# tyb311/TCCT

Measured on AMD Instinct MI355X. Metric: OCT B-scans/sec fwd+bwd(+clip+AdamW), stc_tt bs=8 1x800x1100, higher is better.
Workload: dtype bf16; 1 GPU; stc_tt --los=di bs=8/GPU 1x800x1100 (net tensors 3x800x1104); global_batch=8, parallelism=dp1, ranks=1, grad_allreduce=none, slowest_step=88

## Files before the change

include/tcct_hip.h:

```cpp
#ifndef TCCT_HIP_H
#define TCCT_HIP_H
#include <stdint.h>
#ifdef __cplusplus
extern "C" {
#endif

typedef void* tcct_stream_t;

enum { TCCT_F32 = 0, TCCT_BF16 = 1 };
enum { TCCT_ACT_NONE = 0, TCCT_ACT_LRELU = 1, TCCT_ACT_HSWISH = 2, TCCT_ACT_GELU = 3, TCCT_ACT_SIGMOID = 4,
       TCCT_ACT_ABS = 5 };
enum { TCCT_CRIT_DICE = 0, TCCT_CRIT_DICE2 = 1, TCCT_CRIT_IOU = 2, TCCT_CRIT_MSE = 3 };
enum { TCCT_MCRIT_DICE = 0, TCCT_MCRIT_DICE2 = 1, TCCT_MCRIT_IOU = 2, TCCT_MCRIT_CE = 3 };

int tcct_version(void);
const char* tcct_last_error(void);
int tcct_set_outputs_prezeroed(int on);

int tcct_image_to_nhwc4(const float* img, void* out, int N, int Csrc, int H, int Wsrc, int Wdst, int dtype,
                        tcct_stream_t stream);
int tcct_u8_gather2d(const uint8_t* src, uint8_t* dst, int N, int SH, int SW, int C, int sy0, int sx0, int sh, int sw, int DH, int DW,
                     int dy0, int dx0, int dh, int dw, int flipy, int flipx, int mul, int div, int fill, tcct_stream_t stream);
int tcct_onehot_to_index(const int64_t* onehot, uint8_t* lab, int N, int C, int64_t HW, tcct_stream_t stream);
int tcct_labels_to_u8(const int64_t* lab, uint8_t* out, int N, int H, int Wsrc, int Wdst, tcct_stream_t stream);
// ... 129 lines not shown
                              int PW, int xs, int xo, int ds, int dof, int cin_total, int o_off, int i_off, tcct_stream_t stream);
int tcct_conv32x64_fwd33(const void* x, const void* wp, int wps, const float* bias, void* y, int N, int H, int W, double* stats, int pre_act, int force,
                         tcct_stream_t stream);
int tcct_conv32x64_wgrad33(const void* x, const void* dy, float* dw, float* dbias, int N, int H, int W, int force, tcct_stream_t stream);
int tcct_conv64x32_dgrad33(const void* dy, const void* wp_t, int wps, void* dx, int N, int H, int W, int force, tcct_stream_t stream);
int tcct_conv32_wgrad(const void* x, const void* dy, float* dw, float* dbias, int N, int H, int W, int KH, int KW, int PH,
                      int PW, tcct_stream_t stream);
int tcct_conv32_bwd3x3(const void* x, const void* dy, const void* wp_t, const void* dskip, void* dx, float* dw, float* dbias, int N, int H,
                       int W, tcct_stream_t stream);

int tcct_pw_fwd(const void* x, const float* w, const float* bias, void* y, int64_t M, int K, int N, int transposed,
                int out_dtype, tcct_stream_t stream);
int tcct_pw_wgrad(const void* x, const void* dy, float* dw, float* dbias, int64_t M, int K, int N, tcct_stream_t stream);
int tcct_pw_bwd(const void* x, const void* dy, const float* w, const void* res, void* dx, float* dw, float* dbias, int64_t M, int K, int N,
                tcct_stream_t stream);
int tcct_pw_bwd_cat2(const void* x1, const void* x2, const void* dy, const float* w, void* dx1, void* dx2, float* dw, int64_t M, int K, int N,
                     tcct_stream_t stream);
int tcct_pw_bwd_residual2(const void* x, const void* dy, const float* w, const void* res, void* dx_sum, void* dx_plain, float* dw, float* dbias,
                          int64_t M, int K, int N, tcct_stream_t stream);
int64_t tcct_pw_bwd_bn_supported(int K, int N, int post, int red_post, int split);
int tcct_pw_bwd_bn(const void* x, const void* x2, const void* dz, const void* y, const float* coef, int post, const float* w, const void* res,
                   void* dx, void* dx2, float* dw, float* dbias, int64_t M, int K, int N, const void* y_prev, const float* ab_prev,
                   int red_post, double* sums_prev, tcct_stream_t stream);
int tcct_pw_bwd_bn_sums(const void* x, const void* x2, const void* dz, const void* y, const double* sums, int raw, const float* mean_rstd,
                        const float* ab, float* dgamma, float* dbeta, int post, const float* w, const void* res, void* dx, void* dx2, float* dw,
                        float* dbias, int64_t M, int K, int N, const void* y_prev, const float* ab_prev, int red_post, double* sums_prev,
                        tcct_stream_t stream);
int tcct_pw_wgrad_strided(const void* x, const void* dy, int64_t ldy, float* dw, float* dbias, int64_t M, int K, int N,
                          tcct_stream_t stream);
int tcct_pw_fwd_residual(const void* x, const float* w, const float* bias, const void* res, const float* scale, int64_t per_sample,
                         void* y, void* y_plain, int64_t M, int K, int N, tcct_stream_t stream);
int tcct_pw_fwd_bnstats_xaff(const void* y_prev, const float* ab_prev, const float* w, const float* bias, void* y, int64_t M, int K, int N, double* stats,
                             tcct_stream_t stream);
int tcct_pw_bwd_bn_sums_xaff(const void* y_prev, const float* ab_prev, const void* dz, const void* y, const double* sums, int raw, const float* mean_rstd,
                             const float* ab, float* dgamma, float* dbeta, const float* w, const void* res, void* dx, float* dw, float* dbias, int64_t M,
                             int K, int N, int red_post, double* sums_prev, tcct_stream_t stream);
int tcct_pw_fwd_gelu_residual(const void* x1, const float* w, const float* bias, const void* res, const float* scale, int64_t per_sample, void* y,
                              int64_t M, int K, int N, tcct_stream_t stream);
int tcct_pw_bwd_residual2_sum(const void* x, const void* dy_a, const void* dy_b, const float* w, const void* res, void* dx_sum, void* dx_plain, float* dw,
                              float* dbias, int64_t M, int K, int N, tcct_stream_t stream);
int tcct_pw_bwd_lnb(const void* x, const void* dy, const float* w, const void* t, const float* mean_rstd, const float* gamma, const void* res, void* dt,
                    float* dw, float* dbias, float* dgamma, float* dbeta, int64_t M, int K, int N, tcct_stream_t stream);
int tcct_pw_bwd_gelu(const void* x1, const void* dy, const float* w, void* dx1, float* dw, float* dbias, int64_t M, int K, int N, tcct_stream_t stream);
int tcct_pw_dgrad_residual(const void* dy, const float* w, const void* res, void* dx_sum, void* dx_plain, int64_t M, int Nout, int K,
                           tcct_stream_t stream);
int tcct_pw_fwd_cat2(const void* x1, const void* x2, int K1, const float* w, const float* bias, void* y, int64_t M, int K, int N,
                     double* stats, int pre_act, tcct_stream_t stream);
int tcct_pw_fwd_f32_upadd(const void* x, const float* w, const float* bias, float* y, int B, int uH, int uW, int K, int N, const float* up, tcct_stream_t stream);
int tcct_pw_dgrad_split2(const void* dy, const float* w, void* dx1, void* dx2, int K1, int64_t M, int Nout, int K, tcct_stream_t stream);
int tcct_pw_bwd_cat2_bias(const void* x1, const void* x2, const void* dy, const float* w, void* dx1, void* dx2, float* dw, float* dbias, int64_t M,
                          int K, int N, tcct_stream_t stream);
int tcct_tail_compose(const float* w1, const float* b1, const float* w2, const float* b2, float* wc, float* c, tcct_stream_t stream);
int tcct_tail_compose_bwd(const float* w1, const float* b1, const float* w2, const float* dwc, const float* dc, float* dw1, float* db1, float* dw2,
                          float* db2, tcct_stream_t stream);
int tcct_tail_compose3(const float* w1, const float* b1, const float* w2, const float* b2, const float* w3, const float* b3, int C, float* wcc, float* wa,
                       float* wb, float* ccc, tcct_stream_t stream);
int tcct_tail_compose3_bwd(const float* w1, const float* b1, const float* w2, const float* b2, const float* w3, int C, const float* dwa, const float* dwb,
                           const float* dccc, float* dw1, float* db1, float* dw2, float* db2, float* dw3, float* db3, tcct_stream_t stream);
int tcct_pw_fwd_cat2_f32(const void* x1, const void* x2, int K1, const float* w, const float* bias, float* y, int64_t M, int K, int N, tcct_stream_t stream);
int tcct_head_compose(const float* wt, const float* bt, const float* wa, const float* ba, int C, float* wh, float* ch, tcct_stream_t stream);
int tcct_head_compose_bwd(const float* wt, const float* bt, const float* wa, int C, const float* dwh, const float* dch, float* dwt, float* dbt,
                          float* dwa, float* dba, tcct_stream_t stream);
int tcct_pw_wgrad_cat2(const void* x1, const void* x2, int K1, const void* dy, float* dw, float* dbias, int64_t M, int K, int N,
                       tcct_stream_t stream);
int tcct_pw_fwd_bnstats(const void* x, const float* w, const float* bias, void* y, int64_t M, int K, int N, double* stats, int pre_act,
                        tcct_stream_t stream);

int tcct_im2col3x3_c3(const void* x4, void* out, int N, int H, int W, int stride, int dtype, tcct_stream_t stream);
int tcct_c3_fwd(const void* x4, const float* w, const float* bias, void* y, int B, int H, int W, int stride, double* stats, int stat_pre,
                const float* ab, int pre_act, int post_act, tcct_stream_t stream);
int tcct_c3_wgrad(const void* x4, const void* dy, float* dw, float* dbias, int B, int H, int W, int stride, tcct_stream_t stream);
int tcct_c3_bn_fwd_train(const void* x4, const float* w, const float* bias, void* z, int B, int H, int W, int stride, double* sums,
                         const float* gamma, const float* beta, float eps, float momentum, float* running_mean, float* running_var,
                         int64_t* num_batches_tracked, float* mean_rstd, float* ab, int post_act, tcct_stream_t stream);
int tcct_c3_bn_fwd_eval(const void* x4, const float* w, const float* bias, void* z, int B, int H, int W, int stride, const float* ab, int post_act,
                        tcct_stream_t stream);
int tcct_c3_bn_bwd_reduce(const void* x4, const float* w, const float* bias, const void* dz, int B, int H, int W, int stride, const float* ab,
                          double* raw, int post_act, tcct_stream_t stream);
int tcct_c3_bn_bwd_wgrad(const void* x4, const float* w, const float* bias, const void* dz, int B, int H, int W, int stride, const float* coef,
                         float* dw, float* dbias, int post_act, tcct_stream_t stream);
int64_t tcct_c3_bn_bwd_prefetch(int tiles_ahead);
int tcct_c3_bn_bwd_onepass(const void* x4, const float* w, const float* bias, const void* dz, int B, int H, int W, int stride, const float* mean_rstd,
                           const float* ab, float* work, double* sums, float* dw, float* dbias, float* dgamma, float* dbeta, int post_act, tcct_stream_t stream);
int tcct_pw_wgrad_smalln(const void* x, const void* dy, float* dw, float* dbias, int64_t M, int K, int N, int x_dtype,
                         int dy_dtype, tcct_stream_t stream);

int tcct_stream_copy(const void* src, void* dst, int64_t nbytes, tcct_stream_t stream);

int64_t tcct_kernel_census(int which, int reset);
int tcct_marker(int id, tcct_stream_t stream);

int tcct_dwconv3x3_fwd(const void* x, const float* w, const float* bias, void* y, int N, int H, int W, int C,
                       int stride, int add_input, int dtype, tcct_stream_t stream);
int tcct_dwconv3x3_fwd_bnstats(const void* x, const float* w, const float* bias, void* y, int N, int H, int W, int C, int stride,
                               int add_input, double* stats, int dtype, tcct_stream_t stream);
int tcct_dwconv3x3_dgrad(const void* dy, const float* w, void* dx, int N, int H, int W, int C, int stride,
                         int add_input, int dtype, tcct_stream_t stream);
int tcct_dwconv3x3_dgrad_add(const void* dy, const float* w, const void* res, void* dx, int N, int H, int W, int C, int stride,
                             int add_input, int dtype, tcct_stream_t stream);
int tcct_dwconv3x3_wgrad(const void* x, const void* dy, float* dw, float* dbias, int N, int H, int W, int C,
                         int stride, int dtype, tcct_stream_t stream);
int tcct_dwconv3x3_fwd_xaff(const void* x, const float* xab, const float* w, const float* bias, void* y, int N, int H, int W, int C, int stride,
                            double* stats, int dtype, tcct_stream_t stream);
int tcct_dwconv3x3_wgrad_xaff(const void* x, const float* xab, const void* dy, float* dw, float* dbias, int N, int H, int W, int C, int stride, int dtype,
                              tcct_stream_t stream);
int tcct_dwconv3x3_dgrad_bnred(const void* dy, const float* w, const void* y_prev, const float* ab_prev, void* dx, double* raw, int N, int H, int W, int C,
                               int dtype, tcct_stream_t stream);

int tcct_metapool_fwd(const void* x, void* y, int B, int64_t N, int C, int dtype, tcct_stream_t stream);
int tcct_metapool_bwd(const void* dy, void* dx, int B, int64_t N, int C, int dtype, tcct_stream_t stream);
int tcct_metapool_residual_fwd(const void* x, const void* res, const float* scale, void* y, int B, int64_t N, int C, int dtype,
                               tcct_stream_t stream);
int tcct_metapool_scaled_bwd(const void* dy, const float* scale, void* dx, int B, int64_t N, int C, int dtype, tcct_stream_t stream);
int tcct_ln_metapool_residual_fwd(const void* t, void* y, int B, int64_t N, int C, const float* gamma, const float* beta, float eps, const float* scale,
                                  int dtype, tcct_stream_t stream);
int tcct_ln_metapool_residual_ln_fwd(const void* t, void* y, void* y2, int B, int64_t N, int C, const float* gamma, const float* beta, float eps,
                                     const float* scale, const float* gamma2, const float* beta2, float eps2, float* mean_rstd2, int dtype, tcct_stream_t stream);
int tcct_ln_metapool_residual_bwd(const void* t, const void* dy, void* dt, int B, int64_t N, int C, const float* gamma, float eps, const float* scale,
                                  float* dgamma, float* dbeta, int dtype, tcct_stream_t stream);
int tcct_maxpool2_fwd(const void* x, void* y, int N, int H, int W, int C, int dtype, tcct_stream_t stream);
int tcct_maxpool2_bwd(const void* x, const void* dy, void* dx, int N, int H, int W, int C, int dtype, tcct_stream_t stream);
int tcct_maxpool2_bwd_add(const void* x, const void* dy, const void* res, void* dx, int N, int H, int W, int C, int dtype,
                          tcct_stream_t stream);
int tcct_bilinear_fwd(const void* x, void* y, int N, int H, int W, int C, int Ho, int Wo, int align_corners, int dtype,
                      tcct_stream_t stream);
int tcct_bilinear_bwd_separable(const float* dy, float* dx, float* workspace, int N, int H, int W, int C, int Ho, int Wo,
                                int align_corners, tcct_stream_t stream);
int tcct_bilinear_add_fwd(const void* x, const void* res, void* y, int N, int H, int W, int C, int Ho, int Wo, int align_corners,
                          int dtype, tcct_stream_t stream);
int64_t tcct_bilinear_bwd_x2(int on);
int tcct_bilinear_bwd(const void* dy, void* dx, int N, int H, int W, int C, int Ho, int Wo, int align_corners, int dtype,
                      tcct_stream_t stream);
int tcct_l2norm_fwd(const void* x, void* y, int64_t M, int C, float eps, int dtype, tcct_stream_t stream);
int tcct_l2norm_bwd(const void* x, const void* dy, void* dx, int64_t M, int C, float eps, int dtype, tcct_stream_t stream);
int tcct_l2norm_bwd_scaled(const void* x, const void* dy, void* dx, int64_t M, int C, float eps, float scale, int dtype,
                           tcct_stream_t stream);
int tcct_l2norm_bwd_scaled_add(const void* x, const void* dy, const void* res, void* dx, int64_t M, int C, float eps, float scale, int dtype,
                               tcct_stream_t stream);
int tcct_normadd_fwd(const void* g0, const void* g1, const void* g2, float* inv1, float* inv2, void* out, int N, int H, int W, int C,
                     int h1, int w1, int h2, int w2, float eps, int dtype, tcct_stream_t stream);
int tcct_normadd6_fwd(const void* a0, const void* b0, const void* a1, const void* b1, const void* a2, const void* b2, float* inv1, float* inv2,
                      void* out, int N, int H, int W, int C, int h1, int w1, int h2, int w2, float eps, int dtype, tcct_stream_t stream);
int tcct_l2norm_bwd2_scaled(const void* xa, const void* xb, const void* dn, const void* res_a, const void* res_b, void* da, void* db,
                            int64_t M, int C, float eps, float scale, int dtype, tcct_stream_t stream);

int tcct_softmax_dice_fwd(const void* logits, const uint8_t* labels, int64_t M, int C, double* sums, float* loss,
                          int dtype, tcct_stream_t stream);
int tcct_softmax_dice_bwd(const void* logits, const uint8_t* labels, int64_t M, int C, const double* sums,
                          const float* grad_out, float grad_scale, void* dlogits, int dtype, tcct_stream_t stream);
int tcct_updice_fwd(const float* low, const uint8_t* labels, int B, int h, int w, int H, int W, int C, double* sums, float* loss,
                    tcct_stream_t stream);
int tcct_updice_bwd(const float* low, const uint8_t* labels, int B, int h, int w, int H, int W, int C, const double* sums,
                    const float* grad_out, float grad_scale, float* ws, float* dlow, tcct_stream_t stream);
int tcct_dice_ds_fwd(const void* logits, int dtype, const uint8_t* labels, int B, int H, int W, int C, const float* low1, int h1, int w1, const float* low2,
                     int h2, int w2, const float* low3, int h3, int w3, float coff, double* sums, float* loss, tcct_stream_t stream);
int tcct_softmax_crit_fwd(const void* logits, const uint8_t* labels, int64_t M, int C, int kind, const float* class_w, double* sums, float* loss, int dtype,
                          tcct_stream_t stream);
int tcct_softmax_crit_bwd(const void* logits, const uint8_t* labels, int64_t M, int C, int kind, const float* class_w, const double* sums, const float* grad_out,
                          float grad_scale, void* dlogits, int dtype, tcct_stream_t stream);
int tcct_upcrit_fwd(const float* low, const uint8_t* labels, int B, int h, int w, int H, int W, int C, int kind, const float* class_w, double* sums, float* loss,
                    tcct_stream_t stream);
int tcct_upcrit_bwd(const float* low, const uint8_t* labels, int B, int h, int w, int H, int W, int C, int kind, const float* class_w, const double* sums,
                    const float* grad_out, float grad_scale, float* ws, float* dlow, tcct_stream_t stream);
int tcct_crit_ds_fwd(const void* logits, int dtype, const uint8_t* labels, int B, int H, int W, int C, const float* low1, int h1, int w1, const float* low2, int h2, int w2,
                     const float* low3, int h3, int w3, float coff, int kind, const float* class_w, double* sums, float* loss, tcct_stream_t stream);
int tcct_softmax_mcrit_fwd(const void* logits, const uint8_t* labels, int B, int64_t HW, int C, int kind, const float* class_w, double* sums, float* loss, int dtype,
                           tcct_stream_t stream);
int tcct_softmax_mcrit_bwd(const void* logits, const uint8_t* labels, int B, int64_t HW, int C, int kind, const float* class_w, const double* sums, const float* grad_out,
                           float grad_scale, void* dlogits, int dtype, tcct_stream_t stream);
int tcct_upmcrit_fwd(const float* low, const uint8_t* labels, int B, int h, int w, int H, int W, int C, int kind, const float* class_w, double* sums, float* loss,
                     tcct_stream_t stream);
int tcct_upmcrit_bwd(const float* low, const uint8_t* labels, int B, int h, int w, int H, int W, int C, int kind, const float* class_w, const double* sums,
                     const float* grad_out, float grad_scale, float* ws, float* dlow, tcct_stream_t stream);
int tcct_mcrit_ds_fwd(const void* logits, int dtype, const uint8_t* labels, int B, int H, int W, int C, const float* low1, int h1, int w1, const float* low2, int h2, int w2,
                      const float* low3, int h3, int w3, float coff, int kind, const float* class_w, double* sums, float* loss, tcct_stream_t stream);
int tcct_softmax_pick(const void* logits, const uint8_t* labels, int64_t M, int C, float* prob_lab, uint8_t* argmax,
                      int dtype, tcct_stream_t stream);
int tcct_confusion_counts(const uint8_t* pred, const uint8_t* labels, int N, int64_t HW, int C, float* out,
                          tcct_stream_t stream);

int tcct_gate_fusion_fwd(const void* x1, const void* x2, const float* field, void* y, int N, int H, int W, int C, int hs, int ws,
                         int dtype, tcct_stream_t stream);
int tcct_gate_fusion_bwd(const void* dy, const float* field, void* dx1, void* dx2, int N, int H, int W, int C, int hs, int ws,
                         int dtype, tcct_stream_t stream);

int tcct_mask_boundaries(const uint8_t* mask, int32_t* out, int N, int H, int W, int C, tcct_stream_t stream);

int tcct_eval_counts(const void* pred, int pred_kind, const uint8_t* labels, int B, int H, int W, int C, int h_valid, int w_valid, int32_t* counts, int32_t* bnd_pred,
                     int32_t* bnd_lab, uint8_t* argmax, tcct_stream_t stream);
int tcct_eval_scores(const int32_t* counts, const int32_t* bnd_pred, const int32_t* bnd_lab, int B, int C, int W, int h_valid, int w_valid, double* table,
                     tcct_stream_t stream);
int tcct_ordered_decode(const void* logits, int kind, int B, int H, int W, int C, int h_valid, int w_valid, void* take_ws, uint8_t* mask, int32_t* bnd,
                        int32_t* changed, int32_t* best, tcct_stream_t stream);
int64_t tcct_layout_decode_ws_bytes(int B, int H, int W, int S, int n_free);
int tcct_layout_decode(const void* pred, int kind, int B, int H, int W, int C, const int* layers, int S, int free_mask, int h_valid, int w_valid, void* ws,
                       uint8_t* mask, int32_t* bnd, int32_t* changed, int32_t* best, uint8_t* state, tcct_stream_t stream);
int tcct_eval_layout_scores(const int32_t* counts, const int32_t* bnd_pred, const int32_t* bnd_lab, int B, int C, int S, int W, int h_valid, int w_valid,
                            double* table, tcct_stream_t stream);
int64_t tcct_layout_marginals_ws_bytes(int B, int H, int W, int S, int n_free);
int tcct_layout_marginals(const void* logits, int kind, int B, int H, int W, int C, const int* layers, int S, int free_mask, int h_valid, int w_valid, float tau,
                          void* ws, float* surf, float* var, float* logz, float* post, tcct_stream_t stream);
int tcct_eval_soft_scores(const float* surf, const float* var, const int32_t* bnd_lab, int B, int S, int W, int h_valid, int w_valid, double* table,
                          tcct_stream_t stream);
int64_t tcct_layout_nll_ws_bytes(int B, int H, int W, int S, int n_free);
int tcct_layout_nll_fwd(const void* logits, int kind, const uint8_t* t, const int32_t* bnd_lab, int B, int H, int W, int C, const int* layers, int S, int free_mask,
                        int h_valid, int w_valid, float tau, void* ws, float* nll, tcct_stream_t stream);
int tcct_layout_nll_bwd(const void* logits, int kind, const uint8_t* t, const int32_t* bnd_lab, int B, int H, int W, int C, const int* layers, int S, int free_mask,
                        int h_valid, int w_valid, float tau, const void* ws, const float* gscale, void* grad, tcct_stream_t stream);
int tcct_layout_nll_reduce(const float* nll, const int32_t* bnd_lab, int B, int S, int W, int h_valid, int w_valid, float* out, tcct_stream_t stream);

int tcct_slice_channels_fwd(const void* x, float* y, int64_t M, int C, int start, int n, int dtype, tcct_stream_t stream);
int tcct_slice_channels_bwd(const float* dy, void* dx, int64_t M, int C, int start, int n, int dtype, tcct_stream_t stream);
int tcct_label_planes(const uint8_t* labels, float* onehot, float* edge, int N, int H, int W, int start, int n,
                      tcct_stream_t stream);
int tcct_gumbel_colsoftmax_fwd(const float* x, const float* eps, float* out, float* stats, int N, int H, int W, int CH,
                               tcct_stream_t stream);
int tcct_gumbel_colsoftmax_bwd(const float* x, const float* eps, const float* stats, const float* dout, float* dx, int N,
                               int H, int W, int CH, tcct_stream_t stream);
int tcct_colsoftmax_fwd(const float* x, float* y, int N, int H, int W, tcct_stream_t stream);
int tcct_colsoftmax_bwd(const float* y, const float* dy, float* dx, int N, int H, int W, tcct_stream_t stream);
int tcct_colwsum_fwd(const float* x, const float* wts, float* out, int N, int H, int W, tcct_stream_t stream);
int tcct_colwsum_bwd(const float* dout, const float* wts, float* dx, int N, int H, int W, tcct_stream_t stream);
int tcct_mse_fwd(const float* a, const float* b, int64_t n, double* acc, float* out, tcct_stream_t stream);
int tcct_mse_bwd(const float* a, const float* b, int64_t n, const float* grad_out, float grad_scale, float* da, float* db,
                 tcct_stream_t stream);

int64_t tcct_fpl_select_workspace_bytes();
int tcct_fpl_select(const void* feat, const uint8_t* labels, const float* prob, int64_t M, int C, void* workspace, uint32_t* counts,
                    uint8_t* binmap, float* pro_sum, int dtype, tcct_stream_t stream);
int tcct_fpl_loss(const float* pro_sum, const uint32_t* counts, const float* buf_grad, int C, float* pro, float* loss, float* dpro_over_n,
                  tcct_stream_t stream);
int tcct_fpl_backward(const uint8_t* labels, const uint8_t* binmap, const float* dpro_over_n, const float* grad_out,
                      float grad_scale, int64_t M, void* dfeat, int dtype, tcct_stream_t stream);
int tcct_l2norm_bwd_fplgrad(const void* x, const uint8_t* labels, const uint8_t* binmap, const float* dpro_over_n, const float* grad_out,
                            float grad_scale, int ncls, const void* res, void* dx, int64_t M, float eps, float scale, int dtype, tcct_stream_t stream);
int tcct_bilinear_bwd_fplgrad(const uint8_t* labels, const uint8_t* binmap, const float* dpro_over_n, const float* grad_out, float grad_scale, int ncls,
                              void* dx, int N, int H, int W, int Ho, int Wo, int align_corners, int dtype, tcct_stream_t stream);
int tcct_l2norm_bwd2_fplgrad(const void* xa, const void* xb, const uint8_t* labels, const uint8_t* binmap, const float* dpro_over_n,
                             const float* grad_out, float grad_scale, int ncls, const void* res_a, const void* res_b, void* da, void* db,
                             int64_t M, float eps, float scale, int dtype, tcct_stream_t stream);

int64_t tcct_fatt_kstats_workspace_bytes(int B, int64_t N, int C);
int tcct_fatt_kstats(const void* qkv, void* workspace, float* stats, int B, int64_t N, int C, int heads, int dtype, tcct_stream_t stream);
int tcct_fatt_ktv(const void* qkv, const float* stats, float* M, int B, int64_t N, int C, int heads, int dtype, tcct_stream_t stream);
int tcct_fatt_dktv(const void* qkv, const void* dout, float* dM, float scale, int B, int64_t N, int C, int heads, int dtype,
                   tcct_stream_t stream);
int tcct_fatt_apply_fwd(const void* qkv, const float* M, const void* cv, void* out, float scale, int B, int64_t N, int C, int heads,
                        int dtype, tcct_stream_t stream);
int tcct_fatt_apply_bwd(const void* qkv, const float* stats, const float* M, const float* dM, const void* cv, const void* dout,
                        void* dqkv, void* dcv, float scale, int B, int64_t N, int C, int heads, int dtype, tcct_stream_t stream);
int tcct_dwk_strided_fwd(const void* x, int64_t ldx, const float* w, const float* bias, void* y, int64_t ldy, int B, int H, int W, int Cg,
                         int K, int flip, int accumulate, int dtype, tcct_stream_t stream);
int tcct_dwk_strided_wgrad(const void* x, int64_t ldx, const void* dy, int64_t ldy, float* dw, float* dbias, int B, int H, int W, int Cg,
                           int K, int dtype, tcct_stream_t stream);

int64_t tcct_hydra_kv_workspace_bytes(int B, int64_t N, int C);
int tcct_hydra_kv(const void* qkv, void* workspace, float* kv, int B, int64_t N, int C, int heads, int dtype, tcct_stream_t stream);
int tcct_hydra_dkv(const void* qkv, const void* dmix, void* workspace, float* dkv, float scale, int B, int64_t N, int C, int heads, int dtype,
                   tcct_stream_t stream);
int tcct_hydra_apply_fwd(const void* qkv, const float* kv, const void* cv, void* mix, float scale, int B, int64_t N, int C, int heads,
                         int dtype, tcct_stream_t stream);
int tcct_hydra_apply_bwd(const void* qkv, const float* kv, const float* dkv, const void* cv, const void* dmix, void* dqkv, void* dcv,
                         float scale, int B, int64_t N, int C, int heads, int dtype, tcct_stream_t stream);

int tcct_grad_sumsq(const float* g, int64_t n, double* acc, tcct_stream_t stream);
int tcct_clip_adamw(float* p, const float* g, float* m, float* v, int64_t n, const double* sumsq, float max_norm,
                    float grad_mul, float lr, double beta1, double beta2, float eps, float weight_decay, int step,
                    float* total_norm_out, tcct_stream_t stream);

int tcct_clip_adamw_dev(float* p, const float* g, float* m, float* v, int64_t n, const double* sumsq, float max_norm,
                        float grad_mul, float* state, double beta1, double beta2, float eps, float weight_decay,
                        float* total_norm_out, tcct_stream_t stream);

int tcct_aug_rowcount(const uint8_t* lab, int* cnt, int N, int SH, int SW, tcct_stream_t stream);
int tcct_aug_plan(const float* u, const int* idx, const int* cnt, const uint8_t* lab, int* plan, int B, int N, int SH, int SW, int h, int w,
                  tcct_stream_t stream);
int tcct_aug_apply(const uint8_t* img, const uint8_t* lab, const int* plan, float* out_img, uint8_t* out_lab, int B, int N, int SH, int SW, int C,
                   int h, int w, tcct_stream_t stream);

#ifdef __cplusplus
}
#endif
#endif
```

tcct_amd/csrc/loss.hip:

```cpp
#include "common.h"

#define LB 256
#define MAXC 5
#define MCNS mc5
#include "loss_classes.inc"
#undef MCNS
#undef MAXC
#define MAXC 8

#define MCNS mc8
#include "loss_classes.inc"
#undef MCNS
#undef MAXC
#define MAXC 16
#define MCNS mc16
#include "loss_classes.inc"
#undef MCNS

#define DICE_BY_C(CALL) (C == 5 ? mc5::CALL : (C <= 8 ? mc8::CALL : mc16::CALL))
#define PICK_BY_C(CALL) (C <= 8 ? mc8::CALL : mc16::CALL)

extern "C" int tcct_softmax_dice_fwd(const void* logits, const uint8_t* labels, int64_t M, int C, double* sums, float* loss, int dtype, tcct_stream_t stream) {
    return DICE_BY_C(tcct_softmax_dice_fwd_impl(logits, labels, M, C, sums, loss, dtype, stream));
}
extern "C" int tcct_softmax_dice_bwd(const void* logits, const uint8_t* labels, int64_t M, int C, const double* sums, const float* grad_out, float grad_scale, void* dlogits, int dtype, tcct_stream_t stream) {
    return DICE_BY_C(tcct_softmax_dice_bwd_impl(logits, labels, M, C, sums, grad_out, grad_scale, dlogits, dtype, stream));
}
extern "C" int tcct_updice_fwd(const float* low, const uint8_t* labels, int B, int h, int w, int H, int W, int C, double* sums, float* loss, tcct_stream_t stream) {
    return DICE_BY_C(tcct_updice_fwd_impl(low, labels, B, h, w, H, W, C, sums, loss, stream));
}
extern "C" int tcct_updice_bwd(const float* low, const uint8_t* labels, int B, int h, int w, int H, int W, int C, const double* sums, const float* grad_out, float grad_scale, float* ws, float* dlow, tcct_stream_t stream) {
    return DICE_BY_C(tcct_updice_bwd_impl(low, labels, B, h, w, H, W, C, sums, grad_out, grad_scale, ws, dlow, stream));
}
extern "C" int tcct_dice_ds_fwd(const void* logits, int dtype, const uint8_t* labels, int B, int H, int W, int C, const float* low1, int h1, int w1,
                                const float* low2, int h2, int w2, const float* low3, int h3, int w3, float coff, double* sums, float* loss,
                                tcct_stream_t stream) {
    const float* lows[3] = {low1, low2, low3};
    const int lh[3] = {h1, h2, h3}, lw[3] = {w1, w2, w3};
    const int nlow = low1 ? (low2 ? (low3 ? 3 : 2) : 1) : 0;
    return DICE_BY_C(tcct_dice_ds_fwd_impl(logits, dtype, labels, B, H, W, C, lows, lh, lw, nlow, coff, sums, loss, stream));
}
extern "C" int tcct_softmax_pick(const void* logits, const uint8_t* labels, int64_t M, int C, float* prob_lab, uint8_t* argmax, int dtype, tcct_stream_t stream) {
    return PICK_BY_C(tcct_softmax_pick_impl(logits, labels, M, C, prob_lab, argmax, dtype, stream));
}
extern "C" int tcct_confusion_counts(const uint8_t* pred, const uint8_t* labels, int N, int64_t HW, int C, float* out, tcct_stream_t stream) {
    return PICK_BY_C(tcct_confusion_counts_impl(pred, labels, N, HW, C, out, stream));
}

template <typename T>
__global__ void k_slice_fwd(const T* __restrict__ x, float* __restrict__ y, int64_t M, int C, int start, int n) {
    for (int64_t i = (int64_t)blockIdx.x * blockDim.x + threadIdx.x; i < M * n; i += (int64_t)gridDim.x * blockDim.x)
        y[i] = ldf(x + (i / n) * C + start + (i % n));
}
template <typename T>
__global__ void k_slice_bwd(const float* __restrict__ dy, T* __restrict__ dx, int64_t M, int C, int start, int n) {
    for (int64_t i = (int64_t)blockIdx.x * blockDim.x + threadIdx.x; i < M * C; i += (int64_t)gridDim.x * blockDim.x) {
        int c = (int)(i % C) - start;
        stf(dx + i, (c >= 0 && c < n) ? dy[(i / C) * n + c] : 0.f);
    }
}
extern "C" int tcct_slice_channels_fwd(const void* x, float* y, int64_t M, int C, int start, int n, int dtype, tcct_stream_t stream) {
    TCCT_CHECK(start >= 0 && n > 0 && start + n <= C, "slice_channels_fwd: bad range");
    TCCT_DISPATCH(dtype, hipLaunchKernelGGL(k_slice_fwd<T>, dim3(tcct_grid(M * n, LB, 1 << 16)), dim3(LB), 0, (hipStream_t)stream, (const T*)x, y, M, C, start, n));
    TCCT_LAUNCH_OK();
}
extern "C" int tcct_slice_channels_bwd(const float* dy, void* dx, int64_t M, int C, int start, int n, int dtype, tcct_stream_t stream) {
    TCCT_CHECK(start >= 0 && n > 0 && start + n <= C, "slice_channels_bwd: bad range");
    TCCT_DISPATCH(dtype, hipLaunchKernelGGL(k_slice_bwd<T>, dim3(tcct_grid(M * C, LB, 1 << 16)), dim3(LB), 0, (hipStream_t)stream, dy, (T*)dx, M, C, start, n));
    TCCT_LAUNCH_OK();
}

__global__ void k_label_planes(const uint8_t* __restrict__ lab, float* __restrict__ onehot, float* __restrict__ edge, int N,
                               int H, int W, int start, int n) {
    const int64_t total = (int64_t)N * H * W;
    for (int64_t i = (int64_t)blockIdx.x * blockDim.x + threadIdx.x; i < total; i += (int64_t)gridDim.x * blockDim.x) {
        int l = lab[i];
        if (onehot)
            for (int c = 0; c < n; ++c) onehot[i * n + c] = (l == start + c) ? 1.f : 0.f;
        if (edge) {
            int h = (int)((i / W) % H);
            float e = 0.f;
            if (h > 0) {
                int lp = lab[i - W];
                int cnt = 0;
                if (l != lp) { cnt += (l >= start && l < start + n); cnt += (lp >= start && lp < start + n); }
                e = cnt > 0 ? 1.f : 0.f;
            }
            edge[i] = e;
        }
    }
}
extern "C" int tcct_label_planes(const uint8_t* labels, float* onehot, float* edge, int N, int H, int W, int start, int n,
                                 tcct_stream_t stream) {
    hipLaunchKernelGGL(k_label_planes, dim3(tcct_grid((int64_t)N * H * W, LB, 1 << 16)), dim3(LB), 0, (hipStream_t)stream, labels, onehot, edge, N, H, W, start, n);
    TCCT_LAUNCH_OK();
}

#define GSEG 8
__device__ __forceinline__ float gumbel_z(float x, float e) { return x - 0.5f * logf(-logf(e)); }

template <int CH>
__global__ void __launch_bounds__(64 * GSEG)
k_gumbel_fwd(const float* __restrict__ x, const float* __restrict__ eps, float* __restrict__ out,
             float* __restrict__ stats, int N, int H, int W) {
    __shared__ float sm[GSEG][64], sz[GSEG][64];
    const int WC = W * CH;
    const int64_t cols = (int64_t)N * WC;
    const int lane = threadIdx.x & 63, seg = threadIdx.x >> 6;
    const int64_t col = (int64_t)blockIdx.x * 64 + lane;
    const bool ok = col < cols;
    const int64_t cc = ok ? col : 0;
    const int64_t n = cc / WC;
    const int wc = (int)(cc % WC);
    const float* xp = x + n * (int64_t)H * WC + wc;
    const float* ep = eps + n * (int64_t)H * WC + wc;
    const int hs = (H + GSEG - 1) / GSEG;
    const int h0 = seg * hs, h1 = min(H, h0 + hs);
    float m = -INFINITY, Z = 0.f;
    auto zrow = [&](int h) { return gumbel_z(xp[(int64_t)h * WC], ep[(int64_t)h * WC]); };
    int hq = h0;
    for (; hq + 4 <= h1; hq += 4) {
        const float z0 = zrow(hq), z1 = zrow(hq + 1), z2 = zrow(hq + 2), z3 = zrow(hq + 3);
        const float mn = fmaxf(fmaxf(m, fmaxf(z0, z1)), fmaxf(z2, z3));
        if (mn > -INFINITY) Z = Z * __expf(m - mn) + ((__expf(z0 - mn) + __expf(z1 - mn)) + (__expf(z2 - mn) + __expf(z3 - mn)));
        m = mn;
    }
    for (int h = hq; h < h1; ++h) {
        float z = gumbel_z(xp[(int64_t)h * WC], ep[(int64_t)h * WC]);
        float mn = fmaxf(m, z);
        if (mn > -INFINITY) Z = Z * __expf(m - mn) + __expf(z - mn);
        m = mn;
    }
    sm[seg][lane] = m; sz[seg][lane] = Z;
    __syncthreads();
    m = -INFINITY;
#pragma unroll
    for (int g = 0; g < GSEG; ++g) m = fmaxf(m, sm[g][lane]);
    Z = 0.f;
#pragma unroll
    for (int g = 0; g < GSEG; ++g) if (sm[g][lane] > -INFINITY) Z += sz[g][lane] * __expf(sm[g][lane] - m);
    __syncthreads();
    const float S = 1.f;
    if (ok && seg == 0) { stats[cc * 3] = m; stats[cc * 3 + 1] = Z; stats[cc * 3 + 2] = S; }
    const float den = 1.f / (1e-6f + S);
    for (hq = h0; hq + 4 <= h1; hq += 4) {
        float v[4] = {zrow(hq), zrow(hq + 1), zrow(hq + 2), zrow(hq + 3)};
#pragma unroll
        for (int j = 0; j < 4; ++j) {
            v[j] = __expf(v[j] - m) / Z * den;
#pragma unroll
            for (int o = CH >> 1; o > 0; o >>= 1) v[j] += __shfl_xor(v[j], o, 64);
            if (ok && (wc % CH) == 0) out[(n * H + hq + j) * (int64_t)W + wc / CH] = v[j];
        }
    }
    for (int h = hq; h < h1; ++h) {
// ... 241 lines not shown
```

tcct_amd/csrc/loss_classes.inc:

```
namespace MCNS {
#include "loss_device.inc"
__device__ __forceinline__ void dice_accum(float (&z)[MAXC], int C, int l, float (&I)[MAXC], float (&P)[MAXC], float (&G)[MAXC]) {
    softmax_inplace(z, C);
#pragma unroll
    for (int c = 0; c < MAXC; ++c) {
        P[c] += z[c];
        if (c == l) { I[c] += z[c]; G[c] += 1.f; }
    }
}
#define DSB 1024
template <typename T>
__global__ void __launch_bounds__(DSB) k_dice_sums(const T* __restrict__ logits, const uint8_t* __restrict__ lab, int64_t M, int C,
                            double* __restrict__ sums ) {
    float I[MAXC], P[MAXC], G[MAXC];
#pragma unroll
    for (int c = 0; c < MAXC; ++c) I[c] = P[c] = G[c] = 0.f;
    for (int64_t i = (int64_t)blockIdx.x * blockDim.x + threadIdx.x; i < M; i += (int64_t)gridDim.x * blockDim.x) {
        float z[MAXC];
#pragma unroll
        for (int c = 0; c < MAXC; ++c) z[c] = c < C ? ldf(logits + i * C + c) : -INFINITY;
        dice_accum(z, C, lab[i], I, P, G);
    }
    sums_block_tail<DSB>(I, P, G, C, sums);
}
__global__ void k_dice_finalize(const double* __restrict__ sums, int C, float* __restrict__ loss) {
    if (threadIdx.x == 0) {
        double l = 0.0;
        for (int c = 0; c < C; ++c) l += 1.0 - (1.0 + 2.0 * sums[c]) / (1.0 + sums[C + c] + sums[2 * C + c]);
        *loss = (float)l;
    }
}
static int tcct_softmax_dice_fwd_impl(const void* logits, const uint8_t* labels, int64_t M, int C, double* sums, float* loss,
                                     int dtype, tcct_stream_t stream) {
    TCCT_CHECK(C >= 2 && C <= MAXC, "softmax_dice_fwd: C=%d unsupported (2..%d)", C, MAXC);
    hipStream_t st = (hipStream_t)stream;
    if (hipMemsetAsync(sums, 0, sizeof(double) * 3 * C, st) != hipSuccess) { tcct_set_error("softmax_dice_fwd: memset failed"); return -2; }
    TCCT_DISPATCH(dtype, hipLaunchKernelGGL(k_dice_sums<T>, dim3(tcct_grid(M, DSB, 512)), dim3(DSB), 0, st, (const T*)logits, labels, M, C, sums));
    hipLaunchKernelGGL(k_dice_finalize, dim3(1), dim3(64), 0, st, sums, C, loss);
    TCCT_LAUNCH_OK();
}

__device__ __forceinline__ void dice_grad_coeffs(const double* __restrict__ sums, int C, float (&ka)[MAXC], float (&kb)[MAXC]) {
    __shared__ float s_k[2 * MAXC];
    if ((int)threadIdx.x < C) {
        const int c = threadIdx.x;
        const double U = 1.0 + sums[C + c] + sums[2 * C + c];
        s_k[c] = (float)(-2.0 / U);
        s_k[MAXC + c] = (float)((1.0 + 2.0 * sums[c]) / (U * U));
    }
    __syncthreads();
#pragma unroll
    for (int c = 0; c < MAXC; ++c) { ka[c] = c < C ? s_k[c] : 0.f; kb[c] = c < C ? s_k[MAXC + c] : 0.f; }
}

template <typename T>
__global__ void k_dice_bwd(const T* __restrict__ logits, const uint8_t* __restrict__ lab, int64_t M, int C,
                           const double* __restrict__ sums, const float* __restrict__ gout, float gscale,
                           T* __restrict__ dlogits) {
    float a[MAXC], b[MAXC];
    const float gs = gscale * (gout ? *gout : 1.f);
    dice_grad_coeffs(sums, C, a, b);
    for (int64_t i = (int64_t)blockIdx.x * blockDim.x + threadIdx.x; i < M; i += (int64_t)gridDim.x * blockDim.x) {
        float z[MAXC], mx = -INFINITY;
#pragma unroll
        for (int c = 0; c < MAXC; ++c) { z[c] = c < C ? ldf(logits + i * C + c) : -INFINITY; mx = fmaxf(mx, z[c]); }
        float s = 0.f;
#pragma unroll
        for (int c = 0; c < MAXC; ++c) { z[c] = c < C ? __expf(z[c] - mx) : 0.f; s += z[c]; }
        float inv = __builtin_amdgcn_rcpf(s);
        int l = lab[i];
        float dp[MAXC], dot = 0.f;
#pragma unroll
        for (int c = 0; c < MAXC; ++c) { z[c] *= inv; dp[c] = b[c] + (c == l ? a[c] : 0.f); dot += z[c] * dp[c]; }
#pragma unroll
        for (int c = 0; c < MAXC; ++c)
            if (c < C) stf(dlogits + i * C + c, gs * z[c] * (dp[c] - dot));
    }
}
static int tcct_softmax_dice_bwd_impl(const void* logits, const uint8_t* labels, int64_t M, int C, const double* sums,
                                     const float* grad_out, float grad_scale, void* dlogits, int dtype, tcct_stream_t stream) {
    TCCT_CHECK(C >= 2 && C <= MAXC, "softmax_dice_bwd: C=%d unsupported", C);
    TCCT_DISPATCH(dtype, hipLaunchKernelGGL(k_dice_bwd<T>, dim3(tcct_grid(M, LB, 1 << 16)), dim3(LB), 0, (hipStream_t)stream, (const T*)logits, labels, M, C, sums, grad_out, grad_scale, (T*)dlogits));
    TCCT_LAUNCH_OK();
}

template <int S>
__global__ void __launch_bounds__(UDB) k_updice_sums(const float* __restrict__ low, const uint8_t* __restrict__ lab, int B, int h, int w,
                                                     int H, int W, int C, float sh, double* __restrict__ sums) {
    float I[MAXC], P[MAXC], G[MAXC];
#pragma unroll
    for (int c = 0; c < MAXC; ++c) I[c] = P[c] = G[c] = 0.f;
    const int items = B * H * w;
    const uint32_t m_w = w > 1 ? (uint32_t)((1ull << 32) / (uint32_t)w) : 0xffffffffu, m_H = H > 1 ? (uint32_t)((1ull << 32) / (uint32_t)H) : 0xffffffffu;
    for (int base = blockIdx.x * UDB + (threadIdx.x & ~63); base < items; base += gridDim.x * UDB) {
        const bool live = base + (int)(threadIdx.x & 63) < items;
        const int it = live ? base + (int)(threadIdx.x & 63) : items - 1;
        const int row = (int)udiv32(it, w, m_w), j = it - row * w;
        const int n = (int)udiv32(row, H, m_H), ho = row - n * H;
        float R[3][MAXC];
        updice_rows<S>(low, n, h, w, C, src_index(ho, sh, h, 0), j, R, live);
        if (!live) continue;
        const uint8_t* lr = lab + (int64_t)row * W + S * j;
#pragma unroll
        for (int k = 0; k < S; ++k) {
            float z[MAXC];
            updice_pixel<S>(R, k + S / 2, C, z);
            dice_accum(z, C, lr[k], I, P, G);
        }
    }
    sums_block_tail<UDB>(I, P, G, C, sums);
}
static int dice_launch_upsums(const char* what, const float* low, const uint8_t* labels, int B, int h, int w, int H, int W, int C, double* sums, hipStream_t st) {
    int Sc;
    if (int rc = upsampled_args_ok(what, B, h, w, H, W, &Sc)) return rc;
    UPDICE_SCALES(Sc, hipLaunchKernelGGL(k_updice_sums<S>, dim3(tcct_grid((int64_t)B * H * w, UDB, 512)), dim3(UDB), 0, st, low, labels, B, h, w, H, W, C, (float)h / (float)H, sums));
    return 0;
}
static int tcct_updice_fwd_impl(const float* low, const uint8_t* labels, int B, int h, int w, int H, int W, int C, double* sums,
                               float* loss, tcct_stream_t stream) {
    TCCT_CHECK(C >= 2 && C <= MAXC, "updice_fwd: C=%d unsupported (2..%d)", C, MAXC);
    hipStream_t st = (hipStream_t)stream;
    if (hipMemsetAsync(sums, 0, sizeof(double) * 3 * C, st) != hipSuccess) { tcct_set_error("updice_fwd: memset failed"); return -2; }
    if (int rc = dice_launch_upsums("updice_fwd", low, labels, B, h, w, H, W, C, sums, st)) return rc;
    hipLaunchKernelGGL(k_dice_finalize, dim3(1), dim3(64), 0, st, sums, C, loss);
    TCCT_LAUNCH_OK();
}
template <int S>
__global__ void __launch_bounds__(256) k_updice_bwd_w(const float* __restrict__ low, const uint8_t* __restrict__ lab, int B, int h, int w,
                                                      int H, int W, int C, float sh, const double* __restrict__ sums,
                                                      const float* __restrict__ gout, float gscale, float* __restrict__ T) {
    float ka[MAXC], kb[MAXC];
    const float gs = gscale * (gout ? *gout : 1.f);
    dice_grad_coeffs(sums, C, ka, kb);
    const int lane = threadIdx.x & 63;
    const int wpr = (w + 61) / 62;
    const int nwaves = B * H * wpr;
    const uint32_t m_p = wpr > 1 ? (uint32_t)((1ull << 32) / (uint32_t)wpr) : 0xffffffffu, m_H = H > 1 ? (uint32_t)((1ull << 32) / (uint32_t)H) : 0xffffffffu;
    for (int wv = blockIdx.x * 4 + (int)(threadIdx.x >> 6); wv < nwaves; wv += gridDim.x * 4) {
        const int row = (int)udiv32(wv, wpr, m_p), wir = wv - row * wpr;
        const int n = (int)udiv32(row, H, m_H), ho = row - n * H;
        const int jj = 62 * wir - 1 + lane;
        const bool live = jj >= 0 && jj < w;
        const int j = live ? jj : (jj < 0 ? 0 : w - 1);
        const Lerp a = src_index(ho, sh, h, 0);
        float R[3][MAXC];
        updice_rows<S>(low, n, h, w, C, a, j, R, live);
        float own[MAXC], tlo[MAXC], thi[MAXC];
#pragma unroll
        for (int c = 0; c < MAXC; ++c) own[c] = tlo[c] = thi[c] = 0.f;
        if (live) {
            const uint8_t* lr = lab + (int64_t)row * W + S * j;
#pragma unroll
            for (int k = 0; k < S; ++k) {
                const float f = ((float)k + 0.5f) / (float)S;
                const bool left = k < S / 2;
                const float l1 = left ? f + 0.5f : f - 0.5f, l0 = 1.f - l1;
                float z[MAXC];
                updice_pixel<S>(R, k + S / 2, C, z);
                softmax_inplace(z, C);
                const int l = lr[k];
                float dp[MAXC], dot = 0.f;
#pragma unroll
                for (int c = 0; c < MAXC; ++c) { dp[c] = kb[c] + (c == l ? ka[c] : 0.f); dot += z[c] * dp[c]; }
                const float w_own = left ? (j == 0 ? 1.f : l1) : (j == w - 1 ? 1.f : l0);
                const float w_oth = left ? (j == 0 ? 0.f : l0) : (j == w - 1 ? 0.f : l1);
#pragma unroll
                for (int c = 0; c < MAXC; ++c) {
                    const float g = gs * z[c] * (dp[c] - dot);
                    own[c] += w_own * g;
                    if (left) tlo[c] += w_oth * g; else thi[c] += w_oth * g;
                }
            }
        }
#pragma unroll
        for (int c = 0; c < MAXC; ++c) {
            const float from_left = __shfl_up(thi[c], 1, 64), from_right = __shfl_down(tlo[c], 1, 64);
            own[c] = (from_left + own[c]) + from_right;
        }
        if (live && lane >= 1 && lane <= 62) {
            float* t = T + ((int64_t)row * w + j) * C;
#pragma unroll
            for (int c = 0; c < MAXC; ++c)
                if (c < C) t[c] = own[c];
        }
    }
}
static int tcct_updice_bwd_impl(const float* low, const uint8_t* labels, int B, int h, int w, int H, int W, int C, const double* sums,
                               const float* grad_out, float grad_scale, float* ws, float* dlow, tcct_stream_t stream) {
    TCCT_CHECK(C >= 2 && C <= MAXC, "updice_bwd: C=%d unsupported", C);
    int Sc;
    if (int rc = upsampled_args_ok("updice_bwd", B, h, w, H, W, &Sc)) return rc;
    TCCT_CHECK(ws != nullptr, "updice_bwd: workspace [B,H,w,C] fp32 is NULL");
    hipStream_t st = (hipStream_t)stream;
    UPDICE_SCALES(Sc, hipLaunchKernelGGL(k_updice_bwd_w<S>, dim3(tcct_grid((int64_t)B * H * ((w + 61) / 62), 4, 1 << 14)), dim3(256), 0, st, low, labels, B, h, w, H, W, C, (float)h / (float)H,
                                         sums, grad_out, grad_scale, ws));
    launch_updice_bwd_h(ws, B, h, w, C, H, Sc, dlow, st);
    TCCT_LAUNCH_OK();
}

template <typename T>
__global__ void k_softmax_pick(const T* __restrict__ logits, const uint8_t* __restrict__ lab, int64_t M, int C,
                               float* __restrict__ prob_lab, uint8_t* __restrict__ argmax) {
    for (int64_t i = (int64_t)blockIdx.x * blockDim.x + threadIdx.x; i < M; i += (int64_t)gridDim.x * blockDim.x) {
        float z[MAXC], mx = -INFINITY;
        int am = 0;
#pragma unroll
        for (int c = 0; c < MAXC; ++c) {
            z[c] = c < C ? ldf(logits + i * C + c) : -INFINITY;
            if (z[c] > mx) { mx = z[c]; am = c; }
        }
        if (argmax) argmax[i] = (uint8_t)am;
        if (prob_lab) {
            float s = 0.f, pl = 0.f;
            int l = lab[i];
#pragma unroll
            for (int c = 0; c < MAXC; ++c) { float e = c < C ? __expf(z[c] - mx) : 0.f; s += e; if (c == l) pl = e; }
            prob_lab[i] = pl / s;
        }
    }
}
static int tcct_softmax_pick_impl(const void* logits, const uint8_t* labels, int64_t M, int C, float* prob_lab,
                                 uint8_t* argmax, int dtype, tcct_stream_t stream) {
    TCCT_CHECK(C >= 2 && C <= MAXC, "softmax_pick: C=%d unsupported", C);
    TCCT_CHECK(!(prob_lab && !labels), "softmax_pick: prob_lab needs labels");
    TCCT_DISPATCH(dtype, hipLaunchKernelGGL(k_softmax_pick<T>, dim3(tcct_grid(M, LB, 1 << 16)), dim3(LB), 0, (hipStream_t)stream, (const T*)logits, labels, M, C, prob_lab, argmax));
    TCCT_LAUNCH_OK();
}

__global__ void k_confusion(const uint8_t* __restrict__ pred, const uint8_t* __restrict__ lab, int64_t HW, int C,
                            float* __restrict__ out ) {
    __shared__ float sm[3 * MAXC];
    const int n = blockIdx.y;
    if (threadIdx.x < 3 * MAXC) sm[threadIdx.x] = 0.f;
    __syncthreads();
    float I[MAXC], P[MAXC], G[MAXC];
#pragma unroll
    for (int c = 0; c < MAXC; ++c) I[c] = P[c] = G[c] = 0.f;
    for (int64_t i = (int64_t)blockIdx.x * blockDim.x + threadIdx.x; i < HW; i += (int64_t)gridDim.x * blockDim.x) {
        int p = pred[n * HW + i], l = lab[n * HW + i];
#pragma unroll
        for (int c = 0; c < MAXC; ++c) { P[c] += (p == c); G[c] += (l == c); I[c] += (p == c && l == c); }
    }
#pragma unroll
    for (int c = 0; c < MAXC; ++c) {
        float a = wave_sum(I[c]), b = wave_sum(P[c]), g = wave_sum(G[c]);
        if ((threadIdx.x & 63) == 0) { atomicAdd(&sm[c * 3], a); atomicAdd(&sm[c * 3 + 1], b); atomicAdd(&sm[c * 3 + 2], g); }
    }
    __syncthreads();
    if (threadIdx.x < 3 * C) atomicAdd(&out[(int64_t)n * C * 3 + threadIdx.x], sm[threadIdx.x]);
}
static int tcct_confusion_counts_impl(const uint8_t* pred, const uint8_t* labels, int N, int64_t HW, int C, float* out,
                                     tcct_stream_t stream) {
    TCCT_CHECK(C >= 1 && C <= MAXC, "confusion_counts: C=%d unsupported", C);
    hipStream_t st = (hipStream_t)stream;
    if (hipMemsetAsync(out, 0, sizeof(float) * N * C * 3, st) != hipSuccess) { tcct_set_error("confusion_counts: memset failed"); return -2; }
    dim3 grid(tcct_grid(HW, LB, 256), N);
    hipLaunchKernelGGL(k_confusion, grid, dim3(LB), 0, st, pred, labels, HW, C, out);
    TCCT_LAUNCH_OK();
}

__global__ void k_dice_finalize_ds(const double* __restrict__ sums, int C, int nheads, float coff, float* __restrict__ loss) {
    if (threadIdx.x == 0) {
        float t = 0.f;
        for (int i = nheads - 1; i >= 0; --i) {
            const double* sm = sums + (size_t)i * 3 * C;
            double l = 0.0;
            for (int c = 0; c < C; ++c) l += 1.0 - (1.0 + 2.0 * sm[c]) / (1.0 + sm[C + c] + sm[2 * C + c]);
            t = i > 0 ? t + (float)l * coff : t + (float)l;
        }
        *loss = t;
    }
}
static int tcct_dice_ds_fwd_impl(const void* logits, int dtype, const uint8_t* labels, int B, int H, int W, int C, const float* const* lows, const int* lh,
                                 const int* lw, int nlow, float coff, double* sums, float* loss, tcct_stream_t stream) {
    TCCT_CHECK(C >= 2 && C <= MAXC && nlow >= 0 && nlow <= 3, "dice_ds_fwd: C=%d (2..%d), %d low-resolution heads (0..3)", C, MAXC, nlow);
    hipStream_t st = (hipStream_t)stream;
    if (hipMemsetAsync(sums, 0, sizeof(double) * 3 * C * (1 + nlow), st) != hipSuccess) { tcct_set_error("dice_ds_fwd: memset failed"); return -2; }
    const int64_t M = (int64_t)B * H * W;
    TCCT_DISPATCH(dtype, hipLaunchKernelGGL(k_dice_sums<T>, dim3(tcct_grid(M, DSB, 512)), dim3(DSB), 0, st, (const T*)logits, labels, M, C, sums));
    for (int i = 0; i < nlow; ++i)
        if (int rc = dice_launch_upsums("dice_ds_fwd", lows[i], labels, B, lh[i], lw[i], H, W, C, sums + (size_t)(i + 1) * 3 * C, st)) return rc;
    hipLaunchKernelGGL(k_dice_finalize_ds, dim3(1), dim3(64), 0, st, sums, C, 1 + nlow, coff, loss);
    TCCT_LAUNCH_OK();
}
}
```

Baseline: 425.8 B-scans/s.

## Fuse upsampled dice backward into row-banded kernel and vectorize C=5 dice bwd

Adds a banded upsampled-dice backward kernel. Each wave walks a band of low-res rows, accumulates the vertical interpolation weights in registers and writes dlow directly. This removes the fp32 [B,H,w,C] workspace round-trip and the separate H-direction reduction kernel. Also adds a float4-vectorized fp32 softmax-dice backward for C=5 that processes four pixels per thread. Both paths are on by default and controlled by the TCCT_UPDICE_BWD env var. The risk is lower parallelism, since band rows are serialized per wave, plus recomputation of the boundary rows shared between bands.

Result: no change. 427.1 B-scans/s, median of 6 (+0.3%).

```diff
diff --git a/include/tcct_hip.h b/include/tcct_hip.h
--- a/include/tcct_hip.h
+++ b/include/tcct_hip.h
@@ -305,6 +305,7 @@
                     tcct_stream_t stream);
 int tcct_updice_bwd(const float* low, const uint8_t* labels, int B, int h, int w, int H, int W, int C, const double* sums,
                     const float* grad_out, float grad_scale, float* ws, float* dlow, tcct_stream_t stream);
+int64_t tcct_updice_bwd_banded(int mode);
 int tcct_dice_ds_fwd(const void* logits, int dtype, const uint8_t* labels, int B, int H, int W, int C, const float* low1, int h1, int w1, const float* low2,
                      int h2, int w2, const float* low3, int h3, int w3, float coff, double* sums, float* loss, tcct_stream_t stream);
 int tcct_softmax_crit_fwd(const void* logits, const uint8_t* labels, int64_t M, int C, int kind, const float* class_w, double* sums, float* loss, int dtype,
diff --git a/tcct_amd/csrc/loss.hip b/tcct_amd/csrc/loss.hip
--- a/tcct_amd/csrc/loss.hip
+++ b/tcct_amd/csrc/loss.hip
@@ -1,6 +1,21 @@
 #include "common.h"
+#include <cstdlib>
 
 #define LB 256
+static int g_updice_bwd = -1;
+static int updice_bwd_mode() {
+    if (g_updice_bwd < 0) {
+        const char* e = getenv("TCCT_UPDICE_BWD");
+        const int v = e && *e ? atoi(e) : 1;
+        g_updice_bwd = v >= 0 && v <= 32 ? v : 1;
+    }
+    return g_updice_bwd;
+}
+extern "C" int64_t tcct_updice_bwd_banded(int mode) {
+    const int old = updice_bwd_mode();
+    if (mode >= 0 && mode <= 32) g_updice_bwd = mode;
+    return old;
+}
 #define MAXC 5
 #define MCNS mc5
 #include "loss_classes.inc"
diff --git a/tcct_amd/csrc/loss_classes.inc b/tcct_amd/csrc/loss_classes.inc
--- a/tcct_amd/csrc/loss_classes.inc
+++ b/tcct_amd/csrc/loss_classes.inc
@@ -77,9 +77,63 @@
             if (c < C) stf(dlogits + i * C + c, gs * z[c] * (dp[c] - dot));
     }
 }
+__device__ __forceinline__ void dice_bwd_pixel(float (&z)[MAXC], int l, const float (&a)[MAXC], const float (&b)[MAXC], float gs) {
+    float mx = -INFINITY;
+#pragma unroll
+    for (int c = 0; c < MAXC; ++c) mx = fmaxf(mx, z[c]);
+    float s = 0.f;
+#pragma unroll
+    for (int c = 0; c < MAXC; ++c) { z[c] = __expf(z[c] - mx); s += z[c]; }
+    float inv = __builtin_amdgcn_rcpf(s);
+    float dp[MAXC], dot = 0.f;
+#pragma unroll
+    for (int c = 0; c < MAXC; ++c) { z[c] *= inv; dp[c] = b[c] + (c == l ? a[c] : 0.f); dot = fmaf(z[c], dp[c], dot); }
+#pragma unroll
+    for (int c = 0; c < MAXC; ++c) z[c] = gs * z[c] * (dp[c] - dot);
+}
+__global__ void __launch_bounds__(LB) k_dice_bwd_quad(const float* __restrict__ logits, const uint8_t* __restrict__ lab, int64_t M,
+                                                      const double* __restrict__ sums, const float* __restrict__ gout, float gscale, float* __restrict__ dlogits) {
+    float a[MAXC], b[MAXC];
+    const float gs = gscale * (gout ? *gout : 1.f);
+    dice_grad_coeffs(sums, MAXC, a, b);
+    const int64_t Q = M >> 2;
+    for (int64_t q = (int64_t)blockIdx.x * blockDim.x + threadIdx.x; q < Q; q += (int64_t)gridDim.x * blockDim.x) {
+        const float4* src = reinterpret_cast<const float4*>(logits + q * (4 * MAXC));
+        float v[4 * MAXC];
+#pragma unroll
+        for (int k = 0; k < MAXC; ++k) { const float4 t = src[k]; v[4 * k] = t.x; v[4 * k + 1] = t.y; v[4 * k + 2] = t.z; v[4 * k + 3] = t.w; }
+        const uint32_t l4 = *reinterpret_cast<const uint32_t*>(lab + 4 * q);
+#pragma unroll
+        for (int p = 0; p < 4; ++p) {
+            float z[MAXC];
+#pragma unroll
+            for (int c = 0; c < MAXC; ++c) z[c] = v[p * MAXC + c];
+            dice_bwd_pixel(z, (int)((l4 >> (8 * p)) & 255u), a, b, gs);
+#pragma unroll
+            for (int c = 0; c < MAXC; ++c) v[p * MAXC + c] = z[c];
+        }
+        float4* dst = reinterpret_cast<float4*>(dlogits + q * (4 * MAXC));
+#pragma unroll
+        for (int k = 0; k < MAXC; ++k) dst[k] = make_float4(v[4 * k], v[4 * k + 1], v[4 * k + 2], v[4 * k + 3]);
+    }
+    if (blockIdx.x == 0 && (int64_t)threadIdx.x < (M & 3)) {
+        const int64_t i = 4 * Q + threadIdx.x;
+        float z[MAXC];
+#pragma unroll
+        for (int c = 0; c < MAXC; ++c) z[c] = logits[i * MAXC + c];
+        dice_bwd_pixel(z, lab[i], a, b, gs);
+#pragma unroll
+        for (int c = 0; c < MAXC; ++c) dlogits[i * MAXC + c] = z[c];
+    }
+}
 static int tcct_softmax_dice_bwd_impl(const void* logits, const uint8_t* labels, int64_t M, int C, const double* sums,
                                      const float* grad_out, float grad_scale, void* dlogits, int dtype, tcct_stream_t stream) {
     TCCT_CHECK(C >= 2 && C <= MAXC, "softmax_dice_bwd: C=%d unsupported", C);
+    if (updice_bwd_mode() != 0 && dtype == TCCT_F32 && C == MAXC && M >= 1 && (((uintptr_t)logits | (uintptr_t)dlogits) & 15) == 0 && ((uintptr_t)labels & 3) == 0) {
+        hipLaunchKernelGGL(k_dice_bwd_quad, dim3(tcct_grid(M >> 2, LB, 1 << 16)), dim3(LB), 0, (hipStream_t)stream, (const float*)logits, labels, M, sums, grad_out, grad_scale,
+                           (float*)dlogits);
+        TCCT_LAUNCH_OK();
+    }
     TCCT_DISPATCH(dtype, hipLaunchKernelGGL(k_dice_bwd<T>, dim3(tcct_grid(M, LB, 1 << 16)), dim3(LB), 0, (hipStream_t)stream, (const T*)logits, labels, M, C, sums, grad_out, grad_scale, (T*)dlogits));
     TCCT_LAUNCH_OK();
 }
@@ -185,6 +239,90 @@
         }
     }
 }
+template <int S>
+__global__ void __launch_bounds__(256) k_updice_bwd_band(const float* __restrict__ low, const uint8_t* __restrict__ lab, int B, int h, int w,
+                                                         int H, int W, int C, float sh, const double* __restrict__ sums,
+                                                         const float* __restrict__ gout, float gscale, int RB, int nb , float* __restrict__ dlow) {
+    float ka[MAXC], kb[MAXC];
+    const float gs = gscale * (gout ? *gout : 1.f);
+    dice_grad_coeffs(sums, C, ka, kb);
+    const int lane = threadIdx.x & 63;
+    const int wpr = (w + 61) / 62;
+    const int nwaves = B * nb * wpr;
+    for (int wv = blockIdx.x * 4 + (int)(threadIdx.x >> 6); wv < nwaves; wv += gridDim.x * 4) {
+        const int bi = wv / wpr, wir = wv - bi * wpr;
+        const int n = bi / nb, ib = (bi - n * nb) * RB, ie = min(ib + RB, h);
+        const int jj = 62 * wir - 1 + lane;
+        const bool live = jj >= 0 && jj < w;
+        const int j = live ? jj : (jj < 0 ? 0 : w - 1);
+        const bool writer = live && lane >= 1 && lane <= 62;
+        float prev[MAXC], cur[MAXC];
+#pragma unroll
+        for (int c = 0; c < MAXC; ++c) prev[c] = cur[c] = 0.f;
+#pragma unroll 1
+        for (int i = ib; i <= ie; ++i) {
+#pragma unroll 1
+            for (int t = 0; t < S; ++t) {
+                const int ho = S * i - S / 2 + t;
+                if (ho < 0 || ho >= H) continue;
+                const int row = n * H + ho;
+                const Lerp a = src_index(ho, sh, h, 0);
+                float R[3][MAXC];
+                updice_rows<S>(low, n, h, w, C, a, j, R, live);
+                float own[MAXC], tlo[MAXC], thi[MAXC];
+#pragma unroll
+                for (int c = 0; c < MAXC; ++c) own[c] = tlo[c] = thi[c] = 0.f;
+                if (live) {
+                    const uint8_t* lr = lab + (int64_t)row * W + S * j;
+#pragma unroll
+                    for (int k = 0; k < S; ++k) {
+                        const float f = ((float)k + 0.5f) / (float)S;
+                        const bool left = k < S / 2;
+                        const float l1 = left ? f + 0.5f : f - 0.5f, l0 = 1.f - l1;
+                        float z[MAXC];
+                        updice_pixel<S>(R, k + S / 2, C, z);
+                        softmax_inplace(z, C);
+                        const int l = lr[k];
+                        float dp[MAXC], dot = 0.f;
+#pragma unroll
+                        for (int c = 0; c < MAXC; ++c) { dp[c] = kb[c] + (c == l ? ka[c] : 0.f); dot += z[c] * dp[c]; }
+                        const float w_own = left ? (j == 0 ? 1.f : l1) : (j == w - 1 ? 1.f : l0);
+                        const float w_oth = left ? (j == 0 ? 0.f : l0) : (j == w - 1 ? 0.f : l1);
+#pragma unroll
+                        for (int c = 0; c < MAXC; ++c) {
+                            const float g = gs * z[c] * (dp[c] - dot);
+                            own[c] += w_own * g;
+                            if (left) tlo[c] += w_oth * g; else thi[c] += w_oth * g;
+                        }
+                    }
+                }
+                const float wp = (a.i0 == i - 1 ? a.l0 : 0.f) + (a.i1 == i - 1 ? a.l1 : 0.f), wc = (a.i0 == i ? a.l0 : 0.f) + (a.i1 == i ? a.l1 : 0.f);
+#pragma unroll
+                for (int c = 0; c < MAXC; ++c) {
+                    const float from_left = __shfl_up(thi[c], 1, 64), from_right = __shfl_down(tlo[c], 1, 64);
+                    const float T = (from_left + own[c]) + from_right;
+                    prev[c] += wp * T;
+                    cur[c] += wc * T;
+                }
+            }
+            if (i > ib && writer) {
+                float* d = dlow + (((int64_t)n * h + (i - 1)) * w + j) * C;
+#pragma unroll
+                for (int c = 0; c < MAXC; ++c)
+                    if (c < C) d[c] = prev[c];
+            }
+#pragma unroll
+            for (int c = 0; c < MAXC; ++c) { prev[c] = cur[c]; cur[c] = 0.f; }
+        }
+    }
+}
+static int updice_band_rows(int B, int h, int w, int S) {
+    if (MAXC != 5 || S > 4) return 0;
+    const int64_t per = (int64_t)B * ((w + 61) / 62);
+    for (int r = 1; r < 16; ++r)
+        if (per * ((h + r - 1) / r) <= 4096) return r;
+    return 16;
+}
 static int tcct_updice_bwd_impl(const float* low, const uint8_t* labels, int B, int h, int w, int H, int W, int C, const double* sums,
                                const float* grad_out, float grad_scale, float* ws, float* dlow, tcct_stream_t stream) {
     TCCT_CHECK(C >= 2 && C <= MAXC, "updice_bwd: C=%d unsupported", C);
@@ -192,6 +330,13 @@
     if (int rc = upsampled_args_ok("updice_bwd", B, h, w, H, W, &Sc)) return rc;
     TCCT_CHECK(ws != nullptr, "updice_bwd: workspace [B,H,w,C] fp32 is NULL");
     hipStream_t st = (hipStream_t)stream;
+    const int mode = MAXC == 16 && Sc == 16 ? 0 : updice_bwd_mode();
+    if (const int RB = mode == 1 ? updice_band_rows(B, h, w, Sc) : mode) {
+        const int nb = (h + RB - 1) / RB;
+        UPDICE_SCALES(Sc, if constexpr (MAXC < 16 || S < 16) hipLaunchKernelGGL(k_updice_bwd_band<S>, dim3(tcct_grid((int64_t)B * nb * ((w + 61) / 62), 4, 1 << 14)), dim3(256), 0, st, low, labels, B, h, w, H, W, C,
+                                             (float)h / (float)H, sums, grad_out, grad_scale, RB, nb, dlow));
+        TCCT_LAUNCH_OK();
+    }
     UPDICE_SCALES(Sc, hipLaunchKernelGGL(k_updice_bwd_w<S>, dim3(tcct_grid((int64_t)B * H * ((w + 61) / 62), 4, 1 << 14)), dim3(256), 0, st, low, labels, B, h, w, H, W, C, (float)h / (float)H,
                                          sums, grad_out, grad_scale, ws));
     launch_updice_bwd_h(ws, B, h, w, C, H, Sc, dlow, st);
```
